# ALLabMTL/marl-demandresponse

Measured on AMD Instinct MI355X. Metric: house-steps/s (env.step throughput) at 1M houses; % HBM roofline, higher is better.
Workload: dtype f64; 1 GPU; 1,048,576 houses per GPU, random actions, fused FSM+thermal+reward step, every tick's reward row written (BASELINE metric at 1M houses; configs[1]'s controller); houses_per_gpu=1048576, houses_total=1048576, signal=sinusoidals, penalty=individual_L2, action_mode=random, chunk_ticks=128, window_ticks=32, parallelism=1 GPU

## Files before the change

### include/mdr.h

```cpp
#ifndef MDR_H_
#define MDR_H_

#include <stdint.h>

#ifdef __cplusplus
extern "C" {
#endif

#define MDR_ABI_VERSION 5
#define MDR_MAX_CAP 64

enum {
  MDR_OK = 0,
  MDR_EARG = -1,
  MDR_EHIP = -2,
  MDR_ERCCL = -3,
  MDR_ENOMEM = -4,
  MDR_ESTATE = -5,
};

enum { MDR_PEN_INDIVIDUAL_L2 = 0, MDR_PEN_COMMON_L2 = 1, MDR_PEN_COMMON_MAX = 2, MDR_PEN_MIXTURE = 3 };

enum {
  MDR_ACT_BUFFER = 0,
// ... 44 lines not shown
  double solar;
  double s_prev;
  uint64_t tick;
} mdr_tick;

typedef struct mdr_ctx mdr_ctx;

int mdr_abi_version(void);
const char* mdr_build_id(void);
int mdr_abi_sizes(int64_t* out, int n);
const char* mdr_last_error(void);
int mdr_graph_info(mdr_ctx* ctx, int64_t* out, int n);
int mdr_graph_memset_probe(mdr_ctx* ctx, int64_t* out, int n, void* stream);
int mdr_create(mdr_ctx** out, const mdr_config* cfg);
int mdr_destroy(mdr_ctx* ctx);
int mdr_bind(mdr_ctx* ctx, const mdr_soa* soa);

int mdr_params_changed(mdr_ctx* ctx);

enum { MDR_OPT_STEP_TPW = 1, MDR_OPT_FASTDIV = 2, MDR_OPT_WINDOW_PIPELINE = 3, MDR_OPT_SHARDED_OVERLAP = 4,
       MDR_OPT_GREEDY_SORT = 5, MDR_OPT_FORCE_HALO = 6, MDR_OPT_WINDOW_THERMAL = 7,
       MDR_OPT_HALO_OVERLAP = 9, MDR_OPT_ACTOR_GENERIC = 10, MDR_OPT_HALO_IN_COUNTS = 12,
       MDR_OPT_GQ_BAND = 13, MDR_OPT_ACTOR_FP32_FORM = 14, MDR_OPT_GQ_FUSED = 15, MDR_OPT_GQ_ADAPTIVE = 16,
       MDR_OPT_ACTOR_GRID = 17 };
enum { MDR_FP32_F16_SPLIT = 0, MDR_FP32_BF16_SPLIT3 = 1 };
enum { MDR_THERMAL_EXACT = 0, MDR_THERMAL_AFFINE = 1 };
int mdr_set_option(mdr_ctx* ctx, int option, int64_t value);

size_t mdr_window_onb_bytes(int64_t n_local, int waves);
int mdr_window_geometry_check(int64_t n_local, size_t onb_bytes, size_t wah_bytes);
size_t mdr_window_pen_bytes(int64_t n_local);
int mdr_window_pen_check(int64_t n_local, size_t pen_bytes);
size_t mdr_window_stats_bytes(int64_t n_local);
int mdr_window_stats_check(int64_t n_local, size_t bytes);

typedef struct mdr_pop_spec {
  double target_temp, std_target;
  double thermo_lo, thermo_hi;
  double ca, cm, hm;
  double init_air, init_mass;
  int32_t n_draw;
  uint8_t draw_idx[MDR_MAX_CAP];
} mdr_pop_spec;
int mdr_populate(mdr_ctx* ctx, const mdr_pop_spec* spec, void* stream);

int mdr_power_counts(mdr_ctx* ctx, const uint8_t* action, int action_mode, uint64_t tick,
                     void* stream);
int mdr_counts_buffer(mdr_ctx* ctx, int64_t** dev_ptr, int* len);

int mdr_step(mdr_ctx* ctx, const uint8_t* action, int action_mode, const mdr_tick* tick,
             double* reward, int lookahead, int ctrl, uint8_t* ctrl_out, double* p_out,
             void* stream);

// ... 199 lines not shown
```

### marl-demandresponse_amd/csrc/mdr_capi.hip

```cpp
#include <hip/hip_ext.h>
#include <hip/hip_runtime.h>
#include <hipcub/hipcub.hpp>
#include <rccl/rccl.h>

#include <cmath>
#include <cstdio>
#include <cstdlib>
#include <cstring>
#include <map>
#include <string>
#include <tuple>
#include <vector>

#include "mdr_actor.h"
#include "mdr_devbuf.h"
#include "mdr_interp.h"
#include "mdr_obs_dev.h"
#include "mdr_kernels.h"
#include "mdr_validity.h"

using namespace mdr;

namespace {

// ... 90 lines not shown
  Dev<double> d_partial2;
  Dev<double> d_wpen;
  Dev<double> d_wres;
  Dev<double> d_wstat;
  Dev<double> d_stat_p;
  int pen_blocks = 0;
  int tpw = 0;
  bool fastdiv = true;
  bool win_pipe = true;
  bool tick_overlap = true;
  bool greedy_sort = false;
  bool force_halo = false;
  bool actor_generic = false;
  int actor_grid = 0;
  bool actor_fp32_bf16 = false;
  bool halo_overlap = true;
  bool halo_in_counts = true;
  Dev<unsigned long long> d_c5;
  int thermal = MDR_THERMAL_AFFINE;
  int win = kWindowMax;
  Dev<unsigned long long> d_wslab;
  int wslab_len = 0;
  Dev<uint64_t> d_onb;
  Dev<uint32_t> d_wah;
  Dev<uint64_t> d_onb2;
  Dev<uint32_t> d_wah2;
  Dev<int> d_flags;
  Dev<unsigned> d_tickets;
  Dev<TickArgs> d_ticks;
  std::map<GraphKey, std::pair<hipGraphExec_t, int>> graphs;
  int64_t g_cap = 0;
  Dev<double> g_key, g_key2, g_ps, g_incl;
  Dev<int> g_idx, g_idx2;
  Dev<uint8_t> g_ls;
  Dev<unsigned char> g_tmp;
  Dev<int64_t> g_kpos, g_extra;
  Dev<double> g_part;
  Dev<unsigned> g_hist;
  Dev<unsigned char> g_sel_rec;
  GqSel* g_sel = nullptr;
  Dev<uint4> g_win;
  Dev<uint32_t> g_map;
  Dev<unsigned> g_tickets;
  Dev<double> g_range;
  Dev<uint4> g_sorted;
  int gq_parts_cap = 0;
// ... 357 lines not shown
  k.p_on = c->d_tables + MDR_MAX_CAP;
  if (c->d_flags.reserve(4) || hipMemset(c->d_flags, 0, 16) != hipSuccess)
    return cleanup(fail(MDR_ENOMEM, "flags"));
  if (c->d_tickets.reserve(kTicketWords) ||
      hipMemset(c->d_tickets, 0, kTicketWords * sizeof(unsigned)) != hipSuccess)
    return cleanup(fail(MDR_ENOMEM, "tickets"));
  if (c->d_eps.reserve(1) || hipMemset(c->d_eps, 0, sizeof(float)) != hipSuccess)
    return cleanup(fail(MDR_ENOMEM, "epsilon"));
  k.params_bad = c->d_flags;
  {
    bool ok = cfg->dt < (1 << 20);
    for (int i = 0; i < cfg->n_cap; ++i) ok = ok && fabs(tab[i]) < 1099511627776.0;
    k.fast_tick_ok = ok ? 1 : 0;
  }
  c->slab_len = kCountShards * cfg->n_cap;
  if (c->d_slab.reserve((size_t)kSlabs * c->slab_len))
    return cleanup(fail(MDR_ENOMEM, "count slabs"));
  if (hipMemset(c->d_slab, 0, kSlabs * c->slab_len * sizeof(unsigned long long)) != hipSuccess)
    return cleanup(fail(MDR_EHIP, "count slabs memset"));
  c->tpw = default_tpw(cfg->n_local);
  if (cfg->n_cap <= kWindowCap) {
    c->wslab_len = kWindowMax * kCountShards * cfg->n_cap + kWindowMax * cfg->n_cap + kWindowMax * kWindowRec;
    const size_t tiles64 = whole_blocks(win_tiles(cfg->n_local) + 1, kCountWaves) * kWinHpt + 1;
    if (c->d_wslab.reserve((size_t)3 * c->wslab_len) || c->d_onb.reserve(tiles64 * kWindowMax) ||
        c->d_wah.reserve((size_t)cfg->n_local + 1))
      return cleanup(fail(MDR_ENOMEM, "window count slabs"));
  } else {
    c->win = 0;
  }
  c->pen_blocks = (int)blocks(cfg->n_local, 512);
  if (c->d_pen_partial.reserve((size_t)2 * c->pen_blocks) || c->d_partial2.reserve(2))
    return cleanup(fail(MDR_ENOMEM, "penalty partials"));
  if (cfg->penalty_mode != MDR_PEN_INDIVIDUAL_L2 && c->d_wslab) {
    if (c->d_wpen.reserve(mdr_window_pen_bytes(cfg->n_local) / sizeof(double)) || c->d_wres.reserve(3 * kWindowMax))
      return cleanup(fail(MDR_ENOMEM, "window penalty partials"));
  }
  for (auto& e : c->ev)
    if (hipEventCreate(&e) != hipSuccess) return cleanup(fail(MDR_EHIP, "event"));
  for (int i = 0; i < kSlabs; ++i)
    if (hipEventCreateWithFlags(&c->ev_k1[i], hipEventDisableTiming) != hipSuccess ||
        hipEventCreateWithFlags(&c->ev_ar[i], hipEventDisableTiming) != hipSuccess)
      return cleanup(fail(MDR_EHIP, "event"));
  if (hipEventCreateWithFlags(&c->ev_pc, hipEventDisableTiming) != hipSuccess)
    return cleanup(fail(MDR_EHIP, "event"));
  if (hipDeviceGetAttribute(&c->n_cu, hipDeviceAttributeMultiprocessorCount, cfg->device) != hipSuccess ||
      c->n_cu < 1)
    c->n_cu = 256;
// ... 47 lines not shown
    case MDR_OPT_WINDOW_PIPELINE: c->win_pipe = value != 0; break;
    case MDR_OPT_SHARDED_OVERLAP: c->tick_overlap = value != 0; break;
    case MDR_OPT_GREEDY_SORT: c->greedy_sort = value != 0; break;
    case MDR_OPT_FORCE_HALO: c->force_halo = value != 0; break;
    case MDR_OPT_HALO_OVERLAP: c->halo_overlap = value != 0; break;
    case MDR_OPT_HALO_IN_COUNTS: c->halo_in_counts = value != 0; break;
    case MDR_OPT_GQ_BAND: c->gq_band = value != 0; break;
    case MDR_OPT_GQ_FUSED:
      if (c->gq_fused != (value != 0)) c->v.map_form_switched();
      c->gq_fused = value != 0;
      break;
    case MDR_OPT_GQ_ADAPTIVE: c->gq_adaptive = value != 0; break;
    case MDR_OPT_ACTOR_GENERIC: c->actor_generic = value != 0; break;
    case MDR_OPT_ACTOR_GRID:
      if (value < 0) return fail(MDR_EARG, "mdr_set_option: ACTOR_GRID must be >= 0");
      c->actor_grid = (int)std::min<int64_t>(value, (int64_t)c->n_cu);
      break;
    case MDR_OPT_ACTOR_FP32_FORM:
      if (value != MDR_FP32_F16_SPLIT && value != MDR_FP32_BF16_SPLIT3)
        return fail(MDR_EARG, "mdr_set_option: ACTOR_FP32_FORM must be MDR_FP32_F16_SPLIT or MDR_FP32_BF16_SPLIT3");
      c->actor_fp32_bf16 = value == MDR_FP32_BF16_SPLIT3;
      c->actor_key.clear();
      break;
    case MDR_OPT_WINDOW_THERMAL:
      if (value != MDR_THERMAL_EXACT && value != MDR_THERMAL_AFFINE)
        return fail(MDR_EARG, "mdr_set_option: WINDOW_THERMAL must be MDR_THERMAL_EXACT or _AFFINE");
      c->thermal = (int)value;
      break;
    default: return fail(MDR_EARG, "mdr_set_option: unknown option");
  }
  HIP_TRY(hipDeviceSynchronize());
  destroy_graphs(c);
  return MDR_OK;
}

int mdr_bind(mdr_ctx* c, const mdr_soa* s) {
  enter_writer(c);
  if (!c || !s) return fail(MDR_EARG, "mdr_bind: null argument");
  if (!s->t_air || !s->t_mass || !s->hvac || !s->ua || !s->ca || !s->cm || !s->hm || !s->target ||
      !s->cap_idx)
    return fail(MDR_EARG, "mdr_bind: null array");
  KParams& k = c->kp;
  k.t_air = s->t_air;
  k.t_mass = s->t_mass;
  k.hvac = s->hvac;
  k.ua = s->ua;
// ... 155 lines not shown
  return c->kp.deadband == 0.0 && c->kp.norm_temp == 1.0 && c->kp.alpha_temp >= 0.0 && !std::signbit(c->kp.alpha_temp) &&
         c->kp.alpha_sig >= 0.0 && !std::signbit(c->kp.alpha_sig) && c->kp.norm_sig > 0.0;
}

static bool win_common(const mdr_ctx* c) { return c->kp.penalty_mode != MDR_PEN_INDIVIDUAL_L2; }

static bool window_geom_ok(const mdr_ctx* c) {
  return c->win > 0 && c->d_wslab && c->kp.n_cap <= kWindowCap && c->kp.L < (1 << 30) && c->kp.dt >= 0 &&
         c->kp.dt <= (1 << 25);
}

static bool window_ok(const mdr_ctx* c, int mode) {
  return window_geom_ok(c) && (win_common(c) ? c->d_wpen != nullptr : true) &&
         (mode == MDR_ACT_RANDOM || mode == MDR_ACT_ALWAYS_ON || mode == MDR_ACT_BUFFER);
}

static bool closed_ok(const mdr_ctx* c, int mode, bool stats = false) {
  return window_geom_ok(c) && (win_common(c) ? !stats && c->d_wpen && c->d_wres : true) &&
         (mode == MDR_ACT_BANGBANG || mode == MDR_ACT_DEADBAND_BANGBANG);
}

static int wslab_clean(mdr_ctx* c, hipStream_t st) {
  if (!c->v.slots_dirty() || !c->d_wslab) return MDR_OK;
  HIP_TRY(hipMemsetAsync(c->d_wslab, 0, 3 * sizeof(unsigned long long) * c->wslab_len, st));
  c->v.slots_cleaned();
  return MDR_OK;
}

static unsigned win_grid(const mdr_ctx* c, int waves = 4) {
  return (unsigned)(whole_blocks(win_tiles(c->kp.n), waves) / waves);
}

extern "C" size_t mdr_window_onb_bytes(int64_t n_local, int waves) {
  if (n_local < 0 || waves < 1) return 0;
  return whole_blocks(win_tiles(n_local), waves) * kWinHpt * kWindowMax * sizeof(uint64_t);
}

extern "C" int mdr_window_geometry_check(int64_t n_local, size_t onb_bytes, size_t wah_bytes) {
  if (n_local < 1) return fail(MDR_EARG, "window launch: no houses");
  const size_t need = std::max(mdr_window_onb_bytes(n_local, kCountWaves), mdr_window_onb_bytes(n_local, 4));
  if (onb_bytes < need)
    return fail(MDR_EARG, "window launch: ON-mask rows of " + std::to_string(onb_bytes) + " B, the launch geometry touches " +
                              std::to_string(need) + " B");
  if (wah_bytes < (size_t)n_local * sizeof(uint32_t))
    return fail(MDR_EARG, "window launch: end-word buffer shorter than the shard");
  return MDR_OK;
}

extern "C" size_t mdr_window_pen_bytes(int64_t n_local) {
  if (n_local < 0) return 0;
  return whole_blocks(win_tiles(n_local), 4) * kWindowMax * 2 * sizeof(double);
}

extern "C" int mdr_window_pen_check(int64_t n_local, size_t pen_bytes) {
  if (n_local < 1) return fail(MDR_EARG, "window launch: no houses for the penalty partial rows");
  const size_t need = mdr_window_pen_bytes(n_local);
  if (pen_bytes < need)
    return fail(MDR_EARG, "window launch: penalty partial rows of " + std::to_string(pen_bytes) +
                              " B, the launch geometry writes " + std::to_string(need) + " B");
  return MDR_OK;
}

extern "C" size_t mdr_window_stats_bytes(int64_t n_local) {
  if (n_local < 0) return 0;
  return whole_blocks(win_tiles(n_local), 4) / 4 * kWindowMax * kStats * sizeof(double);
}

extern "C" int mdr_window_stats_check(int64_t n_local, size_t bytes) {
// ... 81 lines not shown
  } while (0)
#define MDR_SW_K(A, SI, CO)                     \
  do {                                          \
    if (ka) MDR_SW_F(A, SI, true, CO);          \
    else MDR_SW_F(A, SI, false, CO);            \
  } while (0)
#define MDR_SW_S(A)                                  \
  do {                                               \
    if (common) MDR_SW_K(A, false, true);            \
    else if (win_simple(c)) MDR_SW_K(A, true, false); \
    else MDR_SW_K(A, false, false);                  \
  } while (0)
  if (mode == MDR_ACT_RANDOM) MDR_SW_S(MDR_ACT_RANDOM);
  else if (mode == MDR_ACT_ALWAYS_ON) MDR_SW_S(MDR_ACT_ALWAYS_ON);
  else MDR_SW_S(MDR_ACT_BUFFER);
#undef MDR_SW_S
#undef MDR_SW_K
#undef MDR_SW_F
#undef MDR_SW_L
  LAUNCH_CHECK("k_step_window");
  return MDR_OK;
}

struct WinSeq {
  mdr_ctx* c;
  const RolloutArgs& a;
  hipStream_t st;
  WinPlan plan;
  const TickArgs* tk(int w) const { return c->d_ticks + plan.start(w); }
  unsigned long long* slot(int w) const { return c->d_wslab + (size_t)(w % 3) * c->wslab_len; }
  const double* rec(int w) const {
    return reinterpret_cast<const double*>(win_red_ptr(c, slot(w)) + (size_t)kWindowMax * c->kp.n_cap);
  }
  double* p_out(int w) const { return w == plan.count() - 1 ? a.p_out : nullptr; }
  int step(int w, int la, uint64_t* onb, uint32_t* wah, unsigned long long* next, const WinDrv* ka = nullptr) const {
    static const WinDrv none{};
    const int t0 = plan.start(w);
    return launch_step_window(c, a.mode, ka != nullptr, a.act_row(t0), a.act_stride, tk(w), plan.size(w), la, rec(w),
                              a.rew_row(t0), a.rew_stride, onb, wah, next, ka ? *ka : none, st);
  }
  int finish(int w) const {
    if (!win_common(c) || (!a.rew_stride && w + 1 < plan.count())) return MDR_OK;
    return win_pen_finish(c, plan.size(w), a.rew_row(plan.start(w)), a.rew_stride, st);
  }
  int staged_windows(int w0, bool shd) const {
    const int nw = plan.count(), ncap = c->kp.n_cap;
// ... 4 lines not shown
      hipLaunchKernelGGL(k_win_reduce, dim3(K), dim3(64 * ncap), 0, st, c->kp, slot(w), K, tk(w), p_out(w));
      LAUNCH_CHECK("k_win_reduce");
      if (int rc = step(w, w + 1 < nw ? plan.size(w + 1) : 0, c->d_onb, c->d_wah, slot(w + 1))) return rc;
      if (int rc = finish(w)) return rc;
    }
    return MDR_OK;
  }
};

static int win_common_unsharded(const mdr_ctx* c, bool shd) {
  if (!win_common(c) || !shd) return MDR_OK;
  return fail(MDR_EARG, "window launches: common penalty modes on a sharded context need the per-step API");
}

static int window_launches(mdr_ctx* c, const RolloutArgs& a, bool shd, hipStream_t st) {
  if (int rc = win_common_unsharded(c, shd)) return rc;
  const WinSeq s{c, a, st, WinPlan(a.n, c->win)};
  SlotsGuard slots(c->v);
  if (int rc = launch_count(c, a.mode, a.action, a.act_stride, c->d_ticks, 0, s.plan.size(0), s.slot(0), c->d_onb,
                            c->d_wah, nullptr, st, false))
    return rc;
  if (int rc = s.staged_windows(0, shd)) return rc;
  return slots.done();
}

enum FirstCounts {
  kCountNow,
  kBegun,
  kBegunAllreduced
};

static int window_launches_direct(mdr_ctx* c, const RolloutArgs& a, const mdr_tick* host_ticks, FirstCounts first,
                                  hipStream_t st) {
  if (int rc = win_common_unsharded(c, first == kBegunAllreduced)) return rc;
  const WinSeq s{c, a, st, WinPlan(a.n, c->win)};
  const int K = s.plan.size(0), nw = s.plan.count();
  SlotsGuard slots(c->v);
  if (first == kCountNow)
    if (int rc = launch_count(c, a.mode, a.action, a.act_stride, nullptr, host_ticks[0].tick, K, s.slot(0), c->d_onb,
                              c->d_wah, nullptr, st, true))
      return rc;
  WinDrv dv{};
  for (int j = 0; j < K; ++j) {
    const mdr_tick& h = host_ticks[j];
    dv.od_k[j] = h.t_od_prev + 273.0;
    dv.solar[j] = h.solar;
    dv.s_prev[j] = h.s_prev;
    if (fabs(h.t_od_prev) < 1048576.0 && fabs(h.solar) < 1099511627776.0) dv.ok |= 1u << j;
  }
  dv.tick0 = host_ticks[0].tick;
  if (nw == 1) dv.p_out = a.p_out;
  if (first == kBegunAllreduced) dv.red = win_red_ptr(c, s.slot(0));
  if (int rc = s.step(0, nw > 1 ? s.plan.size(1) : 0, c->d_onb, c->d_wah, s.slot(1), &dv)) return rc;
  if (int rc = s.finish(0)) return rc;
  if (a.n > K)
    if (int rc = stage_recs(host_ticks + K, a.n - K, c->d_ticks + K, st)) return rc;
  if (int rc = s.staged_windows(1, false)) return rc;
  return slots.done();
}

static int window_pipeline(mdr_ctx* c, const RolloutArgs& a, hipStream_t st) {
  if (int rc = win_common_unsharded(c, true)) return rc;
  const WinSeq s{c, a, st, WinPlan(a.n, c->win)};
  const int nw = s.plan.count();
  hipStream_t cs = c->comm_stream;
  uint64_t* onbs[2] = {c->d_onb, c->d_onb2};
  uint32_t* wahs[2] = {c->d_wah, c->d_wah2};
  SlotsGuard slots(c->v);
  HIP_TRY(hipEventRecord(c->ev_pc, st));
  HIP_TRY(hipStreamWaitEvent(cs, c->ev_pc, 0));
  for (int w = 0; w < nw; ++w) {
    const int K = s.plan.size(w);
    if (w >= 2) HIP_TRY(hipStreamWaitEvent(cs, c->ev_k1[(w - 2) % kSlabs], 0));
    if (int rc = launch_count(c, a.mode, a.act_row(s.plan.start(w)), a.act_stride, s.tk(w), 0, K, s.slot(w),
                              onbs[w % 2], wahs[w % 2], w == 0 ? nullptr : wahs[(w - 1) % 2], cs, true))
      return rc;
    if (int rc = comm_allreduce(c, win_red_ptr(c, s.slot(w)), (size_t)K * c->kp.n_cap, 0, cs)) return rc;
    HIP_TRY(hipEventRecord(c->ev_ar[w % kSlabs], cs));
    HIP_TRY(hipStreamWaitEvent(st, c->ev_ar[w % kSlabs], 0));
    hipLaunchKernelGGL(k_win_records, dim3(1), dim3(kWindowMax), 0, st, c->kp, s.slot(w), K, s.tk(w), s.p_out(w));
    LAUNCH_CHECK("k_win_records");
    if (int rc = s.step(w, 0, onbs[w % 2], wahs[w % 2], s.slot(w))) return rc;
    HIP_TRY(hipEventRecord(c->ev_k1[w % kSlabs], st));
  }
  return slots.done();
}

static bool pipe_buffers(mdr_ctx* c) {
  if (c->d_onb2 && c->d_wah2) return true;
  if (!c->d_onb2.reserve(c->d_onb.capacity()) && !c->d_wah2.reserve(c->d_wah.capacity())) return true;
  (void)hipGetLastError();
  c->d_onb2.reset(), c->d_wah2.reset();
  return false;
}

static int closed_launches(mdr_ctx* c, const RolloutArgs& a, hipStream_t st, double* stats = nullptr) {
  const bool common = win_common(c);
  if (common && stats) return fail(MDR_ESTATE, "window launch: no stats rows from a common-penalty window");
  if (common && (!c->d_wpen || !c->d_wres)) return fail(MDR_ESTATE, "window launch: no penalty partial rows");
  if (stats && !c->d_wstat) return fail(MDR_ESTATE, "window launch: no stats partial rows");
  double* const wstat = stats ? c->d_wstat : nullptr;
  const WinPlan plan(a.n, c->win);
  const int nw = plan.count(), mode = a.mode;
  const int64_t rew_stride = a.rew_stride;
  const KParams kp = c->kp;
  const int ncap = kp.n_cap;
  const TickArgs* const tk = c->d_ticks;
  unsigned long long* slot = c->d_wslab;
  const double* rec = reinterpret_cast<const double*>(win_red_ptr(c, slot) + (size_t)kWindowMax * ncap);
  const unsigned grid = win_grid(c);
  SlotsGuard slots(c->v);
  for (int w = 0; w < nw; ++w) {
    const int K = plan.size(w), t0 = plan.start(w);
// ... 2093 lines not shown
```

### marl-demandresponse_amd/csrc/mdr_kernels.h

```cpp
#pragma once
#include <hip/hip_runtime.h>
#include <stdint.h>

#include "../../include/mdr.h"

namespace mdr {

constexpr int kCountShards = 64;
constexpr int kWinShards = 16;
constexpr int kCountWaves = 16;
constexpr int kTicketGroups = 64;
constexpr int kTicketWords = 32 * (kTicketGroups + 1);
constexpr int kSlabs = 4;
constexpr int kObsBlock = 128;
constexpr int kActBangBang = 16;
constexpr int kActDeadband = 17;

struct KParams {
  int64_t n, goff, n_global;
  int dt, L, n_cap, penalty_mode;
  double deadband, alpha_temp, alpha_sig, norm_temp, norm_sig;
  double alpha_ind_l2, alpha_common_l2, alpha_common_max;
  uint64_t seed;
  double* t_air;
// ... 95 lines not shown
                            GqfBufs fz, int fpar);
constexpr int kPipeMaxCap = 4;
constexpr int kWindowMax = 32;
constexpr int kWindowCap = 4;
constexpr int kWindowRec = 4;
constexpr int kWinHpt = 2;
struct WinDrv {
  double od_k[kWindowMax];
  double solar[kWindowMax];
  double s_prev[kWindowMax];
  uint64_t tick0;
  double* p_out;
  uint32_t ok;
  const unsigned long long* red;
};
struct WinPen {
  double* part;
  double* sig;
};
template <int ACT, int HPT, bool SIMPLE, bool KA, int FORM, bool COMMON = false>
__global__ void k_step_window(KParams p, const uint8_t* action, int64_t act_stride, const TickArgs* tkp, int K,
                              int la_K, const double* rec, double* reward, int64_t rew_stride, uint64_t* onb,
                              uint32_t* wah, unsigned long long* next_slot, WinDrv dv, WinPen pen);
__global__ void k_win_pen_reduce(const double* part, int ntile, double* res);
__global__ void k_win_reward_common(KParams p, const double* res, const double* sig, int j0, double* reward,
                                    int64_t rew_stride);
template <int CTRL, int HPT, bool STATS = false, bool COMMON = false, class... W>
__global__ void k_step_closed(KParams p, const TickArgs* tkp, int K, double* reward, int64_t rew_stride,
                              unsigned long long* slot, W... wstat);
__global__ void k_closed_reward(KParams p, const double* rec, int j0, double* reward, int64_t rew_stride);
__global__ void k_closed_reward_common(KParams p, const double* res, const double* rec, int j0, double* reward,
                                       int64_t rew_stride);
__global__ void k_win_shard_sum(KParams p, unsigned long long* slot);
__global__ void k_closed_reward_sharded(KParams p, const unsigned long long* red, const TickArgs* tkp, int j0, int nt,
                                        double* reward, int64_t rew_stride, double* p_out);
__global__ void k_reward_finalize_dev(KParams p, const TickArgs* tkp, const unsigned long long* counts,
                                      const double* partial2, double* reward);
__global__ void k_win_reduce(KParams p, unsigned long long* slot, int nt, const TickArgs* tkp, double* p_out);
__global__ void k_win_records(KParams p, unsigned long long* slot, int nt, const TickArgs* tkp, double* p_out);
template <int ACT, int HPT>
__global__ void k_count_window(KParams p, const uint8_t* action, int64_t act_stride, const TickArgs* tkp,
                               uint64_t tick0, int nt, unsigned long long* slot, uint64_t* onb, uint32_t* wah,
                               const uint32_t* w_in, unsigned* ticket);
__global__ void k_probe_stream(KParams p, double* reward);
__global__ void k_refresh(KParams p, int* params_bad);
__global__ void k_div_check(const double* a, const double* b, int64_t n, unsigned long long* mismatches);
// ... 113 lines not shown
```

### marl-demandresponse_amd/csrc/mdr_kernels.hip

```cpp
#include "mdr_kernels.h"

#include <tuple>
#include <type_traits>

#include "mdr_device.h"
#include "mdr_obs_dev.h"

namespace mdr {


__device__ __forceinline__ void count_on(bool on, int cls, int n_cap, unsigned* hist,
                                         unsigned long long* slab) {
  const int lane = threadIdx.x & 63;
  for (int k = 0; k < n_cap; ++k) {
    const unsigned long long m = __ballot(on && cls == k);
    if (lane == 0 && m) atomicAdd(&hist[k], (unsigned)__popcll(m));
  }
  __syncthreads();
  if ((int)threadIdx.x < n_cap) {
    const unsigned v = hist[threadIdx.x];
    if (v) atomicAdd(&slab[(blockIdx.x % kCountShards) * n_cap + threadIdx.x],
                     (unsigned long long)v);
  }
}
// ... 870 lines not shown
    *e = 0ull;
  }
#pragma unroll
  for (int off = 32; off > 0; off >>= 1) v += __shfl_xor(v, off);
  if (q == 0 && c < ncap) {
    win_red(slot, ncap)[j * ncap + c] = v;
    s_red[c] = v;
  }
  __syncthreads();
  if (threadIdx.x == 0) {
    if (tk_j) {
      win_tick_record(p, s_red, tk, p_on, win_rec(slot, ncap) + j * kWinRec, j == nt - 1 ? p_out : nullptr);
    } else {
      win_rec(slot, ncap)[j * kWinRec] = win_power(p, s_red, p_on);
    }
  }
}

__global__ void __launch_bounds__(256) k_win_reduce(KParams p, unsigned long long* __restrict__ slot, int nt,
                                                    const TickArgs* __restrict__ tkp, double* p_out) {
  win_reduce_body(p, slot, nt, tkp ? tkp + blockIdx.x : nullptr, p_out);
}

__global__ void __launch_bounds__(256) k_win_shard_sum(KParams p, unsigned long long* __restrict__ slot) {
  const int j = blockIdx.x, c = threadIdx.x >> 6, q = threadIdx.x & 63, ncap = p.n_cap;
  unsigned long long v = 0;
  if (c < ncap) {
    unsigned long long* e = &slot[((size_t)j * kCountShards + q) * ncap + c];
    v = *e;
    *e = 0ull;
  }
#pragma unroll
  for (int off = 32; off > 0; off >>= 1) v += __shfl_xor(v, off);
  if (q == 0 && c < ncap) win_red(slot, ncap)[j * ncap + c] = v;
}

__global__ void __launch_bounds__(kWinMax) k_win_records(KParams p, unsigned long long* __restrict__ slot, int nt,
                                                         const TickArgs* __restrict__ tkp, double* p_out) {
  const int j = threadIdx.x, ncap = p.n_cap;
  if (j >= nt) return;
  double p_on[kWinCap];
#pragma unroll
  for (int k = 0; k < kWinCap; ++k) p_on[k] = p.p_on[k < ncap ? k : 0];
  const unsigned long long* cnt = win_red(slot, ncap) + j * ncap;
  double* rec = win_rec(slot, ncap) + j * kWinRec;
  if (tkp) win_tick_record(p, cnt, tkp[j], p_on, rec, j == nt - 1 ? p_out : nullptr);
// ... 475 lines not shown
  }

#pragma unroll
  for (int h = 0; h < HPT; ++h)
    if (t.v[h]) {
      const uint32_t i = t.i0 + 64u * h;
      p.t_air[i] = T[h]; p.t_mass[i] = Tm[h]; p.hvac[i] = w_end[h];
    }

  if (la_K > 0) {
    uint64_t cmk[HPT][kWinCap];
    win_classes<HPT>(t, cls, cmk);
    win_run<ACT, HPT>(p, w_end, cmk, t, KA ? nullptr : tkp + K, KA ? dv.tick0 + (uint64_t)K : 0, la_K,
                      ACT == MDR_ACT_BUFFER ? action + (int64_t)K * act_stride : nullptr, act_stride, s_cnt[wv],
                      onb_w);
#pragma unroll
    for (int h = 0; h < HPT; ++h)
      if (t.v[h]) wah[t.i0 + 64u * h] = w_end[h];
    __syncthreads();
    win_flush(p, la_K, s_cnt, next_slot);
  }
}

constexpr int kClosedSums = 8;
constexpr int kClosedTr = 68;
struct ClosedLds {
  double tr[4][kClosedSums + 1][kClosedTr];
  double ws[4][kWinMax][kStats];
};
__device__ __forceinline__ ClosedLds& closed_lds() {
  __shared__ ClosedLds s;
  return s;
}
template <bool STATS> struct ClosedAcc {};
template <> struct ClosedAcc<true> {
  double a[kClosedSums], mx;
  uint32_t n_lock, n_on;
};

__device__ __forceinline__ void closed_acc(ClosedAcc<true>& c, double T, double Tm, double tg, double pen, double N) {
  const double e = T - tg / N;
  const double d = T - tg;
  c.a[0] += e;
  c.a[1] += fabs(e);
  c.mx = fmax(c.mx, e);
  c.a[2] += e * e;
// ... 245 lines not shown
                                                                                    double*, int64_t,
                                                                                    unsigned long long*, double*);


#define MDR_INST_WIN_C(A, SI, KA_, FO, CO)                                                                     \
  template __global__ void k_step_window<A, kWinHpt, SI, KA_, FO, CO>(KParams, const uint8_t*, int64_t,        \
                                                                      const TickArgs*, int, int, const double*, \
                                                                      double*, int64_t, uint64_t*, uint32_t*,  \
                                                                      unsigned long long*, WinDrv, WinPen);
#define MDR_INST_WIN_F(A, SI, KA_, FO) MDR_INST_WIN_C(A, SI, KA_, FO, false)
#define MDR_INST_WIN(A)                                                                                         \
  MDR_INST_WIN_C(A, false, false, MDR_THERMAL_EXACT, true) MDR_INST_WIN_C(A, false, true, MDR_THERMAL_EXACT, true)   \
  MDR_INST_WIN_C(A, false, false, MDR_THERMAL_AFFINE, true) MDR_INST_WIN_C(A, false, true, MDR_THERMAL_AFFINE, true) \
  MDR_INST_WIN_F(A, true, false, MDR_THERMAL_EXACT) MDR_INST_WIN_F(A, false, false, MDR_THERMAL_EXACT)          \
  MDR_INST_WIN_F(A, true, true, MDR_THERMAL_EXACT) MDR_INST_WIN_F(A, false, true, MDR_THERMAL_EXACT)            \
  MDR_INST_WIN_F(A, true, false, MDR_THERMAL_AFFINE) MDR_INST_WIN_F(A, false, false, MDR_THERMAL_AFFINE)        \
  MDR_INST_WIN_F(A, true, true, MDR_THERMAL_AFFINE) MDR_INST_WIN_F(A, false, true, MDR_THERMAL_AFFINE)          \
  template __global__ void k_count_window<A, kWinHpt>(KParams, const uint8_t*, int64_t, const TickArgs*, uint64_t, \
                                                      int, unsigned long long*, uint64_t*, uint32_t*, const uint32_t*, \
                                                      unsigned*);
MDR_INST_WIN(MDR_ACT_RANDOM)
MDR_INST_WIN(MDR_ACT_ALWAYS_ON)
MDR_INST_WIN(MDR_ACT_BUFFER)

#define MDR_INST_PIPE(T, A, LA, G)                                                                    \
  template __global__ void k_step_pipe<T, A, LA, G>(KParams, const uint8_t*, TickArgs, const TickArgs*, \
                                                    const unsigned long long*, double*, double*,         \
                                                    unsigned long long*, unsigned long long*, GqOut, GqfBufs, int);
MDR_INST_PIPE(1, MDR_ACT_RANDOM, MDR_ACT_RANDOM, 0)
MDR_INST_PIPE(2, MDR_ACT_RANDOM, MDR_ACT_RANDOM, 0)
MDR_INST_PIPE(4, MDR_ACT_RANDOM, MDR_ACT_RANDOM, 0)
MDR_INST_PIPE(8, MDR_ACT_RANDOM, MDR_ACT_RANDOM, 0)
MDR_INST_PIPE(2, MDR_ACT_BUFFER, 0, 0)
MDR_INST_PIPE(4, MDR_ACT_BUFFER, 0, 0)
MDR_INST_PIPE(2, MDR_ACT_BUFFER, 0, 1)
MDR_INST_PIPE(4, MDR_ACT_BUFFER, 0, 1)
MDR_INST_PIPE(2, MDR_ACT_BUFFER, 0, 2)
MDR_INST_PIPE(4, MDR_ACT_BUFFER, 0, 2)

#define MDR_INST_STEP(F, A, LA)                                                                  \
  template __global__ void k_step_t<2, F, A, LA>(                                                \
      KParams, const uint8_t*, int, TickArgs, const TickArgs*, const unsigned long long*,        \
      double*, int, uint8_t*, double*, int, unsigned long long*, unsigned long long*, double*, int);
MDR_INST_STEP(false, -1, -1)
MDR_INST_STEP(true, -1, -1)
MDR_INST_STEP(true, MDR_ACT_RANDOM, MDR_ACT_RANDOM)
// ... 2302 lines not shown
```

### marl-demandresponse_amd/mdr_amd/_lib.py

```python
from __future__ import annotations

import ctypes as C
import os
import threading

HERE = os.path.dirname(os.path.abspath(__file__))
LIB_PATH = os.environ.get("MDR_LIB", os.path.join(HERE, "libmdr_hip.so"))

ABI_VERSION = 5
MAX_CAP = 64

ACT_BUFFER, ACT_RANDOM, ACT_ALWAYS_ON, ACT_BANGBANG, ACT_DEADBAND_BANGBANG = 0, 1, 2, 16, 17
CTRL_NONE, CTRL_BANGBANG, CTRL_DEADBAND_BANGBANG, CTRL_GREEDY_KEYS = 0, 1, 2, 3
COMM_RING, COMM_TABLE = 0, 1
PEN_MODES = {"individual_L2": 0, "common_L2": 1, "common_max_error": 2, "mixture": 3}
ERRORS = {-1: "MDR_EARG", -2: "MDR_EHIP", -3: "MDR_ERCCL", -4: "MDR_ENOMEM", -5: "MDR_ESTATE"}
OPTIONS = {"step_tpw": 1, "fastdiv": 2, "window_pipeline": 3, "sharded_overlap": 4, "greedy_sort": 5, "halo_overlap": 9, "actor_generic": 10,
           "force_halo": 6, "window_thermal": 7, "halo_in_counts": 12,
           "gq_band": 13, "actor_fp32_form": 14, "gq_fused": 15, "gq_adaptive": 16, "actor_grid": 17}
THERMAL_EXACT, THERMAL_AFFINE = 0, 1
FP32_F16_SPLIT, FP32_BF16_SPLIT3 = 0, 1
HEADS = {"softmax": 0, "q": 1}


class MdrLibraryError(RuntimeError):
    """libmdr_hip.so is missing or unusable (no CPU fallback exists)."""


class MdrError(RuntimeError):
    pass


class mdr_config(C.Structure):
    _fields_ = [
        ("abi_version", C.c_int32), ("device", C.c_int32),
        ("n_local", C.c_int64), ("global_offset", C.c_int64), ("n_global", C.c_int64),
        ("dt", C.c_int32), ("lockout_duration", C.c_int32),
        ("cop", C.c_double), ("lcf", C.c_double), ("deadband", C.c_double),
        ("n_cap", C.c_int32), ("penalty_mode", C.c_int32),
        ("cap_table", C.c_double * MAX_CAP),
        ("alpha_temp", C.c_double), ("alpha_sig", C.c_double),
        ("norm_temp", C.c_double), ("norm_sig", C.c_double),
# ... 73 lines not shown
P, VP, I, I64, U64, D = C.POINTER, C.c_void_p, C.c_int, C.c_int64, C.c_uint64, C.c_double

HOST_ALLREDUCE_FN = C.CFUNCTYPE(I, VP, VP, I64, I)
HOST_SENDRECV_FN = C.CFUNCTYPE(I, VP, VP, I64, I, VP, I64, I, I)

SIGNATURES = {
    "mdr_abi_version": (I, []),
    "mdr_abi_sizes": (I, [P(I64), I]),
    "mdr_last_error": (C.c_char_p, []),
    "mdr_graph_info": (I, [VP, P(I64), I]),
    "mdr_graph_memset_probe": (I, [VP, P(I64), I, VP]),
    "mdr_actor_status": (I, [VP, P(I64), I, VP]),
    "mdr_actor_set_head": (I, [VP, I, C.c_float, VP]),
    "mdr_greedy_fused_diag": (I, [VP, P(U64)]),
    "mdr_greedy_fused_stamps": (I, [VP, I, P(U64)]),
    "mdr_create": (I, [P(VP), P(mdr_config)]),
    "mdr_destroy": (I, [VP]),
    "mdr_bind": (I, [VP, P(mdr_soa)]),
    "mdr_params_changed": (I, [VP]),
    "mdr_set_rollout_window": (I, [VP, I]),
    "mdr_set_option": (I, [VP, I, I64]),
    "mdr_window_onb_bytes": (C.c_size_t, [I64, I]),
    "mdr_window_geometry_check": (I, [I64, C.c_size_t, C.c_size_t]),
    "mdr_window_pen_bytes": (C.c_size_t, [I64]),
    "mdr_window_pen_check": (I, [I64, C.c_size_t]),
    "mdr_window_stats_bytes": (C.c_size_t, [I64]),
    "mdr_window_stats_check": (I, [I64, C.c_size_t]),
    "mdr_time_step_kernels": (I, [VP, I, VP, VP, I64, I, VP, I64, VP, P(C.c_float), P(I)]),
    "mdr_rollout_begin": (I, [VP, I, U64, VP, I64, I, VP]),
    "mdr_populate": (I, [VP, P(mdr_pop_spec), VP]),
    "mdr_power_counts": (I, [VP, VP, I, U64, VP]),
    "mdr_counts_buffer": (I, [VP, P(VP), P(I)]),
    "mdr_step": (I, [VP, VP, I, P(mdr_tick), VP, I, I, VP, VP, VP]),
    "mdr_penalty_partials": (I, [VP, VP]),
    "mdr_penalty_buffer": (I, [VP, P(VP)]),
    "mdr_reward_finalize": (I, [VP, P(mdr_tick), VP, VP]),
    "mdr_rollout": (I, [VP, I, VP, VP, I64, I, VP, I64, VP, I, VP]),
    "mdr_rollout_stats": (I, [VP, I, VP, VP, I64, I, VP, I64, VP, VP, I, I, VP]),
    "mdr_rollout_stats_path": (I, [VP, I]),
    "mdr_msg_width": (I, [P(mdr_obs_spec)]),
    "mdr_obs": (I, [VP, P(mdr_obs_spec), P(mdr_obs_scalars), VP, VP, VP]),
    "mdr_halo_pack": (I, [VP, P(mdr_obs_spec), VP, VP]),
    "mdr_msg_pack": (I, [VP, P(mdr_obs_spec), VP, VP]),
    "mdr_ctrl_greedy": (I, [VP, D, VP, VP]),
    "mdr_greedy_fallbacks": (I, [VP, VP]),
    "mdr_greedy_diag": (I, [VP, VP]),
# ... 160 lines not shown
```

Baseline: 415.0 billion house-steps/s.

## Group up to four rollout windows per step kernel launch

Adds a grouped window path, on by default with group size 4. It processes several consecutive 32-tick windows in one k_step_group launch and reduces their counts together in k_win_reduce_group. House state (temperatures, parameters, thermal coefficients) is loaded and stored once per group rather than once per window, and the number of kernel launches and reductions drops. In exchange it needs more count-slab slots and ON-mask rows, shared memory for four windows' counts, and serialises four lookahead FSM runs inside one kernel, which may hurt occupancy.

```diff
diff --git a/include/mdr.h b/include/mdr.h
--- a/include/mdr.h
+++ b/include/mdr.h
@@ -90,13 +90,14 @@
        MDR_OPT_GREEDY_SORT = 5, MDR_OPT_FORCE_HALO = 6, MDR_OPT_WINDOW_THERMAL = 7,
        MDR_OPT_HALO_OVERLAP = 9, MDR_OPT_ACTOR_GENERIC = 10, MDR_OPT_HALO_IN_COUNTS = 12,
        MDR_OPT_GQ_BAND = 13, MDR_OPT_ACTOR_FP32_FORM = 14, MDR_OPT_GQ_FUSED = 15, MDR_OPT_GQ_ADAPTIVE = 16,
-       MDR_OPT_ACTOR_GRID = 17 };
+       MDR_OPT_ACTOR_GRID = 17, MDR_OPT_WINDOW_GROUP = 18 };
 enum { MDR_FP32_F16_SPLIT = 0, MDR_FP32_BF16_SPLIT3 = 1 };
 enum { MDR_THERMAL_EXACT = 0, MDR_THERMAL_AFFINE = 1 };
 int mdr_set_option(mdr_ctx* ctx, int option, int64_t value);
 
 size_t mdr_window_onb_bytes(int64_t n_local, int waves);
 int mdr_window_geometry_check(int64_t n_local, size_t onb_bytes, size_t wah_bytes);
+int mdr_window_group_check(int64_t n_local, int windows, size_t onb_bytes, size_t wah_bytes);
 size_t mdr_window_pen_bytes(int64_t n_local);
 int mdr_window_pen_check(int64_t n_local, size_t pen_bytes);
 size_t mdr_window_stats_bytes(int64_t n_local);
diff --git a/marl-demandresponse_amd/csrc/mdr_capi.hip b/marl-demandresponse_amd/csrc/mdr_capi.hip
--- a/marl-demandresponse_amd/csrc/mdr_capi.hip
+++ b/marl-demandresponse_amd/csrc/mdr_capi.hip
@@ -136,6 +136,8 @@
   Dev<unsigned long long> d_wslab;
   int wslab_len = 0;
   Dev<uint64_t> d_onb;
+  size_t onb_rows = 0;
+  int win_group = kWinGroup;
   Dev<uint32_t> d_wah;
   Dev<uint64_t> d_onb2;
   Dev<uint32_t> d_wah2;
@@ -539,7 +541,8 @@
   if (cfg->n_cap <= kWindowCap) {
     c->wslab_len = kWindowMax * kCountShards * cfg->n_cap + kWindowMax * cfg->n_cap + kWindowMax * kWindowRec;
     const size_t tiles64 = whole_blocks(win_tiles(cfg->n_local) + 1, kCountWaves) * kWinHpt + 1;
-    if (c->d_wslab.reserve((size_t)3 * c->wslab_len) || c->d_onb.reserve(tiles64 * kWindowMax) ||
+    c->onb_rows = tiles64 * kWindowMax;
+    if (c->d_wslab.reserve((size_t)kWinSlots * c->wslab_len) || c->d_onb.reserve((1 + kWinGroup) * c->onb_rows) ||
         c->d_wah.reserve((size_t)cfg->n_local + 1))
       return cleanup(fail(MDR_ENOMEM, "window count slabs"));
   } else {
@@ -633,6 +636,10 @@
       c->actor_fp32_bf16 = value == MDR_FP32_BF16_SPLIT3;
       c->actor_key.clear();
       break;
+    case MDR_OPT_WINDOW_GROUP:
+      if (value < 0 || value > kWinGroup) return fail(MDR_EARG, "mdr_set_option: WINDOW_GROUP outside 0..4");
+      c->win_group = (int)value;
+      break;
     case MDR_OPT_WINDOW_THERMAL:
       if (value != MDR_THERMAL_EXACT && value != MDR_THERMAL_AFFINE)
         return fail(MDR_EARG, "mdr_set_option: WINDOW_THERMAL must be MDR_THERMAL_EXACT or _AFFINE");
@@ -834,7 +841,7 @@
 
 static int wslab_clean(mdr_ctx* c, hipStream_t st) {
   if (!c->v.slots_dirty() || !c->d_wslab) return MDR_OK;
-  HIP_TRY(hipMemsetAsync(c->d_wslab, 0, 3 * sizeof(unsigned long long) * c->wslab_len, st));
+  HIP_TRY(hipMemsetAsync(c->d_wslab, 0, kWinSlots * sizeof(unsigned long long) * c->wslab_len, st));
   c->v.slots_cleaned();
   return MDR_OK;
 }
@@ -856,6 +863,18 @@
                               std::to_string(need) + " B");
   if (wah_bytes < (size_t)n_local * sizeof(uint32_t))
     return fail(MDR_EARG, "window launch: end-word buffer shorter than the shard");
+  return MDR_OK;
+}
+
+extern "C" int mdr_window_group_check(int64_t n_local, int windows, size_t onb_bytes, size_t wah_bytes) {
+  if (n_local < 1) return fail(MDR_EARG, "window group launch: no houses");
+  if (windows < 1 || windows > kWinGroup) return fail(MDR_EARG, "window group launch: windows outside 1..4");
+  const size_t need = (size_t)windows * mdr_window_onb_bytes(n_local, 4);
+  if (onb_bytes < need)
+    return fail(MDR_EARG, "window group launch: ON-mask rows of " + std::to_string(onb_bytes) +
+                              " B, the launch geometry touches " + std::to_string(need) + " B");
+  if (wah_bytes < (size_t)n_local * sizeof(uint32_t))
+    return fail(MDR_EARG, "window group launch: end-word buffer shorter than the shard");
   return MDR_OK;
 }
 
@@ -983,6 +1002,50 @@
   return MDR_OK;
 }
 
+static int launch_step_group(mdr_ctx* c, int mode, bool ka, const uint8_t* action, int64_t act_stride,
+                             const TickArgs* tk, const WinGrp& g, double* reward, int64_t rew_stride,
+                             const WinDrv& dv, hipStream_t st) {
+  if (c->d_onb.capacity() < c->onb_rows) return fail(MDR_ESTATE, "window group launch: no group mask rows");
+  if (int rc = mdr_window_group_check(c->kp.n, kWinGroup, dev_bytes(c->d_onb) - c->onb_rows * sizeof(uint64_t),
+                                      dev_bytes(c->d_wah)))
+    return rc;
+  if (g.nw < 1 || g.nw > kWinGroup || g.la_nw < 0 || g.la_nw > kWinGroup)
+    return fail(MDR_EARG, "window group launch: windows outside 1..4");
+  for (int i = 0; i < kWinGroup; ++i)
+    if (g.K[i] < 0 || g.K[i] > kWindowMax || g.la_K[i] < 0 || g.la_K[i] > kWindowMax)
+      return fail(MDR_EARG, "window group launch: a window of more than 32 ticks");
+  const unsigned grid = win_grid(c);
+  const KParams kp = c->kp;
+  uint64_t* onb = c->d_onb + c->onb_rows;
+#define MDR_SG_L(A, SI, KA_, FO)                                                                               \
+  hipLaunchKernelGGL((k_step_group<A, kWinHpt, SI, KA_, FO>), dim3(grid), dim3(256), 0, st, kp, action, act_stride, tk, g, \
+                     reward, rew_stride, onb, (uint32_t*)c->d_wah, dv)
+#define MDR_SG_F(A, SI, KA_)                                                         \
+  do {                                                                               \
+    if (c->thermal == MDR_THERMAL_AFFINE) MDR_SG_L(A, SI, KA_, MDR_THERMAL_AFFINE);  \
+    else MDR_SG_L(A, SI, KA_, MDR_THERMAL_EXACT);                                    \
+  } while (0)
+#define MDR_SG_K(A, SI)              \
+  do {                               \
+    if (ka) MDR_SG_F(A, SI, true);   \
+    else MDR_SG_F(A, SI, false);     \
+  } while (0)
+#define MDR_SG_S(A)                          \
+  do {                                       \
+    if (win_simple(c)) MDR_SG_K(A, true);    \
+    else MDR_SG_K(A, false);                 \
+  } while (0)
+  if (mode == MDR_ACT_RANDOM) MDR_SG_S(MDR_ACT_RANDOM);
+  else if (mode == MDR_ACT_ALWAYS_ON) MDR_SG_S(MDR_ACT_ALWAYS_ON);
+  else MDR_SG_S(MDR_ACT_BUFFER);
+#undef MDR_SG_S
+#undef MDR_SG_K
+#undef MDR_SG_F
+#undef MDR_SG_L
+  LAUNCH_CHECK("k_step_group");
+  return MDR_OK;
+}
+
 struct WinSeq {
   mdr_ctx* c;
   const RolloutArgs& a;
@@ -1033,6 +1096,51 @@
     return rc;
   if (int rc = s.staged_windows(0, shd)) return rc;
   return slots.done();
+}
+
+static int window_groups(const WinSeq& s, int G, const WinDrv& dv, const mdr_tick* host_ticks) {
+  mdr_ctx* c = s.c;
+  const RolloutArgs& a = s.a;
+  const int nw = s.plan.count(), K0 = s.plan.size(0), ncap = c->kp.n_cap;
+  auto slot = [&](int w) { return c->d_wslab + (size_t)(w % kWinSlots) * c->wslab_len; };
+  auto rec = [&](int w) {
+    return reinterpret_cast<const double*>(win_red_ptr(c, slot(w)) + (size_t)kWindowMax * ncap);
+  };
+  auto ahead = [&](WinGrp& g, int w1) {
+    g.la_nw = std::max(0, std::min(G, nw - w1));
+    for (int i = 0; i < g.la_nw; ++i) g.la_K[i] = s.plan.size(w1 + i), g.la_slot[i] = slot(w1 + i);
+  };
+  static const WinDrv none{};
+  {
+    WinGrp g{};
+    g.nw = 1, g.K[0] = K0, g.rec[0] = rec(0), g.first_onb = c->d_onb;
+    ahead(g, 1);
+    if (int rc = launch_step_group(c, a.mode, true, a.act_row(0), a.act_stride, s.tk(0), g, a.rew_row(0), a.rew_stride,
+                                   dv, s.st))
+      return rc;
+  }
+  if (a.n > K0)
+    if (int rc = stage_recs(host_ticks + K0, a.n - K0, c->d_ticks + K0, s.st)) return rc;
+  for (int w = 1; w < nw; w += G) {
+    const int cnt = std::min(G, nw - w), t0 = s.plan.start(w);
+    WinRed r{};
+    WinGrp g{};
+    r.nw = g.nw = cnt;
+    for (int i = 0; i < cnt; ++i) {
+      r.K[i] = g.K[i] = s.plan.size(w + i);
+      r.slot[i] = slot(w + i);
+      r.tk[i] = s.tk(w + i);
+      g.rec[i] = rec(w + i);
+    }
+    r.p_out = w + cnt == nw ? a.p_out : nullptr;
+    hipLaunchKernelGGL(k_win_reduce_group, dim3(r.K[0], cnt), dim3(64 * ncap), 0, s.st, c->kp, r);
+    LAUNCH_CHECK("k_win_reduce_group");
+    ahead(g, w + cnt);
+    if (int rc = launch_step_group(c, a.mode, false, a.act_row(t0), a.act_stride, s.tk(w), g, a.rew_row(t0),
+                                   a.rew_stride, none, s.st))
+      return rc;
+  }
+  return MDR_OK;
 }
 
 enum FirstCounts {
@@ -1062,6 +1170,10 @@
   dv.tick0 = host_ticks[0].tick;
   if (nw == 1) dv.p_out = a.p_out;
   if (first == kBegunAllreduced) dv.red = win_red_ptr(c, s.slot(0));
+  if (c->win_group > 0 && first != kBegunAllreduced && !has_comm(c) && c->world <= 1 && !win_common(c)) {
+    if (int rc = window_groups(s, c->win_group, dv, host_ticks)) return rc;
+    return slots.done();
+  }
   if (int rc = s.step(0, nw > 1 ? s.plan.size(1) : 0, c->d_onb, c->d_wah, s.slot(1), &dv)) return rc;
   if (int rc = s.finish(0)) return rc;
   if (a.n > K)
@@ -1099,7 +1211,7 @@
 
 static bool pipe_buffers(mdr_ctx* c) {
   if (c->d_onb2 && c->d_wah2) return true;
-  if (!c->d_onb2.reserve(c->d_onb.capacity()) && !c->d_wah2.reserve(c->d_wah.capacity())) return true;
+  if (!c->d_onb2.reserve(c->onb_rows) &&!c->d_wah2.reserve(c->d_wah.capacity())) return true;
   (void)hipGetLastError();
   c->d_onb2.reset(), c->d_wah2.reset();
   return false;
diff --git a/marl-demandresponse_amd/csrc/mdr_kernels.h b/marl-demandresponse_amd/csrc/mdr_kernels.h
--- a/marl-demandresponse_amd/csrc/mdr_kernels.h
+++ b/marl-demandresponse_amd/csrc/mdr_kernels.h
@@ -141,6 +141,26 @@
 __global__ void k_step_window(KParams p, const uint8_t* action, int64_t act_stride, const TickArgs* tkp, int K,
                               int la_K, const double* rec, double* reward, int64_t rew_stride, uint64_t* onb,
                               uint32_t* wah, unsigned long long* next_slot, WinDrv dv, WinPen pen);
+constexpr int kWinGroup = 4;
+constexpr int kWinSlots = 2 * kWinGroup;
+struct WinGrp {
+  int nw, la_nw;
+  int K[kWinGroup], la_K[kWinGroup];
+  const double* rec[kWinGroup];
+  unsigned long long* la_slot[kWinGroup];
+  const uint64_t* first_onb;
+};
+template <int ACT, int HPT, bool SIMPLE, bool KA, int FORM>
+__global__ void k_step_group(KParams p, const uint8_t* action, int64_t act_stride, const TickArgs* tkp, WinGrp g,
+                             double* reward, int64_t rew_stride, uint64_t* onb, uint32_t* wah, WinDrv dv);
+struct WinRed {
+  int nw;
+  int K[kWinGroup];
+  unsigned long long* slot[kWinGroup];
+  const TickArgs* tk[kWinGroup];
+  double* p_out;
+};
+__global__ void k_win_reduce_group(KParams p, WinRed r);
 __global__ void k_win_pen_reduce(const double* part, int ntile, double* res);
 __global__ void k_win_reward_common(KParams p, const double* res, const double* sig, int j0, double* reward,
                                     int64_t rew_stride);
diff --git a/marl-demandresponse_amd/csrc/mdr_kernels.hip b/marl-demandresponse_amd/csrc/mdr_kernels.hip
--- a/marl-demandresponse_amd/csrc/mdr_kernels.hip
+++ b/marl-demandresponse_amd/csrc/mdr_kernels.hip
@@ -916,6 +916,12 @@
   win_reduce_body(p, slot, nt, tkp ? tkp + blockIdx.x : nullptr, p_out);
 }
 
+__global__ void __launch_bounds__(256) k_win_reduce_group(KParams p, WinRed r) {
+  const int w = blockIdx.y, K = r.K[w];
+  if ((int)blockIdx.x >= K) return;
+  win_reduce_body(p, r.slot[w], K, r.tk[w] + blockIdx.x, w == r.nw - 1 ? r.p_out : nullptr);
+}
+
 __global__ void __launch_bounds__(256) k_win_shard_sum(KParams p, unsigned long long* __restrict__ slot) {
   const int j = blockIdx.x, c = threadIdx.x >> 6, q = threadIdx.x & 63, ncap = p.n_cap;
   unsigned long long v = 0;
@@ -1437,6 +1443,214 @@
   }
 }
 
+template <int ACT, int HPT, bool SIMPLE, bool KA, int FORM>
+__global__ void __launch_bounds__(256) k_step_group(KParams p, const uint8_t* __restrict__ action,
+                                                    int64_t act_stride, const TickArgs* __restrict__ tkp, WinGrp g,
+                                                    double* __restrict__ reward, int64_t rew_stride,
+                                                    uint64_t* __restrict__ onb, uint32_t* __restrict__ wah,
+                                                    WinDrv dv) {
+  constexpr bool AFF = FORM == MDR_THERMAL_AFFINE;
+  __shared__ unsigned s_cnt[kWinGroup][4][kWinMax * kWinCap];
+  const int wv = threadIdx.x >> 6;
+  const WinTile<HPT> t(p);
+  uint64_t* onb_w = onb + (size_t)t.tile * kWinGroup * HPT * kWinMax;
+  const uint64_t* onb_r = KA ? g.first_onb + (size_t)t.tile * HPT * kWinMax : onb_w;
+  uint32_t ns_lo = 0, ns_hi = 0;
+  if (KA) {
+    const int K = g.K[0];
+    const double* rec = g.rec[0];
+    const int l = (int)(threadIdx.x & 63) < K ? (int)(threadIdx.x & 63) : 0;
+    const double P = rec[l * kWinRec];
+    if (dv.p_out && blockIdx.x == 0 && threadIdx.x == 0) *dv.p_out = rec[(K - 1) * kWinRec];
+    const double ns = win_nsig(p, P, dv.s_prev[l]);
+    ns_lo = (uint32_t)__double_as_longlong(ns);
+    ns_hi = (uint32_t)((uint64_t)__double_as_longlong(ns) >> 32);
+  }
+
+  double T[HPT], Tm[HPT], ua[HPT], hm[HPT], tg[HPT], ca[HPT], cm[HPT];
+  uint32_t w_end[HPT];
+  int cls[HPT];
+  const bool params_ok = !*p.params_bad && p.fast_tick_ok;
+#pragma unroll
+  for (int h = 0; h < HPT; ++h) {
+    const uint32_t i = t.idx[h];
+    T[h] = p.t_air[i]; Tm[h] = p.t_mass[i]; ua[h] = p.ua[i]; hm[h] = p.hm[i]; tg[h] = p.target[i];
+    ca[h] = p.ca[i]; cm[h] = p.cm[i];
+    w_end[h] = wah[i];
+    cls[h] = p.cap_idx[i];
+  }
+  double q_on[kWinCap];
+#pragma unroll
+  for (int c = 0; c < kWinCap; ++c) q_on[c] = p.q_on[c < p.n_cap ? c : 0];
+  double qc[HPT], lo_tg[HPT], hi_tg[HPT];
+#pragma unroll
+  for (int h = 0; h < HPT; ++h) {
+    qc[h] = q_on[0];
+#pragma unroll
+    for (int c = 1; c < kWinCap; ++c) qc[h] = cls[h] == c ? q_on[c] : qc[h];
+    hi_tg[h] = tg[h] + p.deadband / 2.0;
+    lo_tg[h] = tg[h] - p.deadband / 2.0;
+  }
+  RcWin rw[AFF ? 1 : HPT];
+  AffWin aw[AFF ? HPT : 1];
+  double tk[HPT], tmk[HPT], hk[HPT];
+#pragma unroll
+  for (int h = 0; h < HPT; ++h) {
+    if constexpr (AFF) {
+      aw[h] = aff_window(ua[h], ca[h], cm[h], hm[h], (double)p.dt, qc[h], params_ok);
+      hk[h] = hi_tg[h] + 273.0;
+    } else if (params_ok) {
+      rw[h] = rc_window(ua[h], ca[h], cm[h], hm[h], (double)p.dt);
+    } else {
+      rw[h].k = rc_coeffs_t<false>(ua[h], ca[h], cm[h], hm[h], (double)p.dt);
+      rw[h].rCa.nb = -ca[h];
+      rw[h].rc.nb = -ua[h];
+      rw[h].rd.nb = -(rw[h].k.r2 - rw[h].k.r1);
+      rw[h].UaHm = ua[h] + hm[h];
+    }
+  }
+
+  const uint32_t rb = t.i0 * 8u;
+  const double nalpha = -p.alpha_temp;
+  auto lane_nsig = [&](int j) { return __longlong_as_double((long long)readlane_u64(ns_lo, ns_hi, j)); };
+  int tick_off = 0;
+  for (int gi = 0; gi < g.nw; ++gi) {
+    const int K = g.K[gi];
+    const double* __restrict__ rec = g.rec[gi];
+    const uint64_t* onb_g = onb_r + gi * (kWinMax * HPT);
+    bool win_finite = true;
+    if constexpr (AFF) {
+#pragma unroll
+      for (int h = 0; h < HPT; ++h) {
+        tk[h] = T[h] + 273.0;
+        tmk[h] = Tm[h] + 273.0;
+        const AffWin& a = aw[h];
+        const double s = a.tt + a.tm + a.tq + a.to + a.qt + a.mt + a.mm + a.mq + a.mo + a.qm + tk[h] + tmk[h] + hk[h];
+        win_finite = win_finite && (s - s == 0.0);
+      }
+      win_finite = __all(win_finite);
+    }
+
+    double r_od = KA ? dv.od_k[0] : rec[0], r_sol = KA ? dv.solar[0] : rec[1], r_sig = KA ? lane_nsig(0) : rec[2];
+    uint64_t r_ok = KA ? (uint64_t)(dv.ok & 1u) : __double_as_longlong(rec[3]);
+    uint64_t r_on[HPT];
+#pragma unroll
+    for (int h = 0; h < HPT; ++h) r_on[h] = onb_g[h];
+    for (int j = 0; j < K; ++j) {
+      const double od_k = r_od, solar = r_sol, nsig = r_sig;
+      const bool tick_ok = r_ok != 0;
+      uint64_t on_m[HPT];
+#pragma unroll
+      for (int h = 0; h < HPT; ++h) on_m[h] = r_on[h];
+      const int jn = j + 1 < K ? j + 1 : j;
+      if (KA) {
+        r_od = dv.od_k[jn];
+        r_sol = dv.solar[jn];
+        r_sig = lane_nsig(jn);
+        r_ok = (dv.ok >> jn) & 1u;
+      } else {
+        r_od = rec[jn * kWinRec + 0];
+        r_sol = rec[jn * kWinRec + 1];
+        r_sig = rec[jn * kWinRec + 2];
+        r_ok = __double_as_longlong(rec[jn * kWinRec + 3]);
+      }
+#pragma unroll
+      for (int h = 0; h < HPT; ++h) r_on[h] = onb_g[jn * HPT + h];
+      char* rrow = reinterpret_cast<char*>(reward + (int64_t)(tick_off + j) * rew_stride);
+      auto reward_of = [&](int h, double Tn, double tkn, auto fast_c) {
+        constexpr bool F = decltype(fast_c)::value;
+        if (SIMPLE) {
+          if (AFF && F) {
+            const double x = tkn - hk[h];
+            return __builtin_fma(nalpha, x * x, nsig);
+          }
+          const double x = Tn - hi_tg[h];
+          const double pen = F ? x * x : deadband_l2_0(hi_tg[h], Tn);
+          return nalpha * pen + nsig;
+        }
+        double pen = 0.0;
+        if (hi_tg[h] < Tn) { const double x = Tn - hi_tg[h]; pen = x * x; }
+        else if (lo_tg[h] > Tn) { const double x = lo_tg[h] - Tn; pen = x * x; }
+        const double tpen = p.alpha_temp * pen;
+        return -((p.norm_temp == 1.0 ? tpen : tpen / p.norm_temp) + -nsig);
+      };
+      if constexpr (AFF) {
+        auto houses = [&](auto fast_c) {
+#pragma unroll
+          for (int h = 0; h < HPT; ++h) {
+            const AffWin& a = aw[h];
+            const bool on = __builtin_amdgcn_inverse_ballot_w64(on_m[h]);
+            const double ut = __builtin_fma(a.to, od_k, __builtin_fma(a.tq, solar, on ? a.qt : 0.0));
+            const double um = __builtin_fma(a.mo, od_k, __builtin_fma(a.mq, solar, on ? a.qm : 0.0));
+            const double tkn = __builtin_fma(a.tt, tk[h], __builtin_fma(a.tm, tmk[h], ut));
+            const double tmkn = __builtin_fma(a.mt, tk[h], __builtin_fma(a.mm, tmk[h], um));
+            tk[h] = tkn;
+            tmk[h] = tmkn;
+            const double r = reward_of(h, tkn - 273.0, tkn, fast_c);
+            if (t.v[h]) __builtin_nontemporal_store(r, reinterpret_cast<double*>(rrow + (rb + 512u * h)));
+          }
+        };
+        if (win_finite && tick_ok) houses(std::true_type());
+        else houses(std::false_type());
+      } else {
+        uint64_t ok_m = ~0ull;
+#pragma unroll
+        for (int h = 0; h < HPT; ++h)
+          ok_m &= __builtin_amdgcn_ballot_w64(fabs(T[h]) < 1048576.0) & __builtin_amdgcn_ballot_w64(fabs(Tm[h]) < 1048576.0);
+        const bool fast = params_ok && tick_ok && ok_m == __builtin_amdgcn_read_exec();
+        auto houses = [&](auto fast_c) {
+          constexpr bool F = decltype(fast_c)::value;
+#pragma unroll
+          for (int h = 0; h < HPT; ++h) {
+            const bool on = __builtin_amdgcn_inverse_ballot_w64(on_m[h]);
+            const double q = on ? qc[h] : 0.0;
+            double Tn, Tmn;
+            rc_apply_win<F>(T[h], Tm[h], ua[h], hm[h], rw[h], q, solar, od_k, Tn, Tmn);
+            T[h] = Tn;
+            Tm[h] = Tmn;
+            const double r = reward_of(h, Tn, 0.0, fast_c);
+            if (t.v[h]) __builtin_nontemporal_store(r, reinterpret_cast<double*>(rrow + (rb + 512u * h)));
+          }
+        };
+        if (fast) houses(std::true_type());
+        else houses(std::false_type());
+      }
+    }
+    if constexpr (AFF) {
+#pragma unroll
+      for (int h = 0; h < HPT; ++h) {
+        T[h] = tk[h] - 273.0;
+        Tm[h] = tmk[h] - 273.0;
+      }
+    }
+    tick_off += K;
+  }
+
+#pragma unroll
+  for (int h = 0; h < HPT; ++h)
+    if (t.v[h]) {
+      const uint32_t i = t.i0 + 64u * h;
+      p.t_air[i] = T[h]; p.t_mass[i] = Tm[h]; p.hvac[i] = w_end[h];
+    }
+
+  if (g.la_nw > 0) {
+    uint64_t cmk[HPT][kWinCap];
+    win_classes<HPT>(t, cls, cmk);
+    for (int li = 0; li < g.la_nw; ++li) {
+      const int la_K = g.la_K[li];
+      win_run<ACT, HPT>(p, w_end, cmk, t, KA ? nullptr : tkp + tick_off, KA ? dv.tick0 + (uint64_t)tick_off : 0, la_K,
+                        ACT == MDR_ACT_BUFFER ? action + (int64_t)tick_off * act_stride : nullptr, act_stride,
+                        s_cnt[li][wv], onb_w + li * (kWinMax * HPT));
+      tick_off += la_K;
+    }
+#pragma unroll
+    for (int h = 0; h < HPT; ++h)
+      if (t.v[h]) wah[t.i0 + 64u * h] = w_end[h];
+    __syncthreads();
+    for (int li = 0; li < g.la_nw; ++li) win_flush(p, g.la_K[li], s_cnt[li], g.la_slot[li]);
+  }
+}
+
 constexpr int kClosedSums = 8;
 constexpr int kClosedTr = 68;
 struct ClosedLds {
@@ -1728,6 +1942,18 @@
 MDR_INST_WIN(MDR_ACT_RANDOM)
 MDR_INST_WIN(MDR_ACT_ALWAYS_ON)
 MDR_INST_WIN(MDR_ACT_BUFFER)
+
+#define MDR_INST_GRP_F(A, SI, KA_, FO)                                                                         \
+  template __global__ void k_step_group<A, kWinHpt, SI, KA_, FO>(KParams, const uint8_t*, int64_t, const TickArgs*, \
+                                                                 WinGrp, double*, int64_t, uint64_t*, uint32_t*, WinDrv);
+#define MDR_INST_GRP(A)                                                                                    \
+  MDR_INST_GRP_F(A, true, false, MDR_THERMAL_EXACT) MDR_INST_GRP_F(A, false, false, MDR_THERMAL_EXACT)     \
+  MDR_INST_GRP_F(A, true, true, MDR_THERMAL_EXACT) MDR_INST_GRP_F(A, false, true, MDR_THERMAL_EXACT)       \
+  MDR_INST_GRP_F(A, true, false, MDR_THERMAL_AFFINE) MDR_INST_GRP_F(A, false, false, MDR_THERMAL_AFFINE)   \
+  MDR_INST_GRP_F(A, true, true, MDR_THERMAL_AFFINE) MDR_INST_GRP_F(A, false, true, MDR_THERMAL_AFFINE)
+MDR_INST_GRP(MDR_ACT_RANDOM)
+MDR_INST_GRP(MDR_ACT_ALWAYS_ON)
+MDR_INST_GRP(MDR_ACT_BUFFER)
 
 #define MDR_INST_PIPE(T, A, LA, G)                                                                    \
   template __global__ void k_step_pipe<T, A, LA, G>(KParams, const uint8_t*, TickArgs, const TickArgs*, \
diff --git a/marl-demandresponse_amd/mdr_amd/_lib.py b/marl-demandresponse_amd/mdr_amd/_lib.py
--- a/marl-demandresponse_amd/mdr_amd/_lib.py
+++ b/marl-demandresponse_amd/mdr_amd/_lib.py
@@ -17,7 +17,7 @@
 ERRORS = {-1: "MDR_EARG", -2: "MDR_EHIP", -3: "MDR_ERCCL", -4: "MDR_ENOMEM", -5: "MDR_ESTATE"}
 OPTIONS = {"step_tpw": 1, "fastdiv": 2, "window_pipeline": 3, "sharded_overlap": 4, "greedy_sort": 5, "halo_overlap": 9, "actor_generic": 10,
            "force_halo": 6, "window_thermal": 7, "halo_in_counts": 12,
-           "gq_band": 13, "actor_fp32_form": 14, "gq_fused": 15, "gq_adaptive": 16, "actor_grid": 17}
+           "gq_band": 13, "actor_fp32_form": 14, "gq_fused": 15, "gq_adaptive": 16, "actor_grid": 17, "window_group": 18}
 THERMAL_EXACT, THERMAL_AFFINE = 0, 1
 FP32_F16_SPLIT, FP32_BF16_SPLIT3 = 0, 1
 HEADS = {"softmax": 0, "q": 1}
@@ -137,6 +137,7 @@
     "mdr_set_option": (I, [VP, I, I64]),
     "mdr_window_onb_bytes": (C.c_size_t, [I64, I]),
     "mdr_window_geometry_check": (I, [I64, C.c_size_t, C.c_size_t]),
+    "mdr_window_group_check": (I, [I64, I, C.c_size_t, C.c_size_t]),
     "mdr_window_pen_bytes": (C.c_size_t, [I64]),
     "mdr_window_pen_check": (I, [I64, C.c_size_t]),
     "mdr_window_stats_bytes": (C.c_size_t, [I64]),
```

After: 428.4 billion house-steps/s, median of 6. +3.2%, better.
